# arihantb2/direct_lidar_odometry

Hardware: AMD Instinct MI355X
Metric: gicp_iterations_per_sec (higher is better)
Workload: dtype f64

## Files before the change

### direct_lidar_odometry_amd/csrc/ngicp_align.h

```cpp
#pragma once

namespace {

std::mutex& persist_mutex(int device) {
  static std::mutex m[64];
  return m[(unsigned)device % 64u];
}

int pass_impl() {
  static const int impl = std::getenv("NGICP_PASS_IMPL") ? std::atoi(std::getenv("NGICP_PASS_IMPL")) : 0;
  return impl;
}

const char* robust_unsupported_switch(const ngicp* h) {
  if (pass_impl() == 1) return "NGICP_PASS_IMPL=1";
  if (const char* s = std::getenv("NGICP_FUSED")) if (std::atoi(s) != 0) return "NGICP_FUSED";
  if (const char* s = std::getenv("NGICP_QUEUE")) if (std::atoi(s) != 0) return "NGICP_QUEUE";
  if (h->persist) return "NGICP_PERSIST";
  if (h->head) return "NGICP_HEAD";
  return nullptr;
}
void refuse_if_robust(const ngicp* h, const char* entry) {
  if (h->robust_kind != NGICP_ROBUST_NONE)
    throw ArgError{NGICP_ERR_ARG, std::string(entry) + ": not available with a robust kernel set (ngicp_set_robust_kernel(h, NGICP_ROBUST_NONE, 0) turns it off)"};
// ... 164 lines not shown
  s.partials = a.partials;
  s.nblocks = nblocks;
  s.grp_order = order_buf[h->order_sel];
  s.grp_cost = a.grp_cost;
  s.trace = own_buffers ? h->trace.as<double>() : nullptr;
  s.max_trace_rows = max_rows;
  s.mode = 0;
  s.sums_out = nullptr;
  s.dbg_stamps = nullptr;
  s.progress_host = nullptr;
  s.final_host = nullptr;
  s.order_valid = order_flag[h->order_sel];
  s.t_first = nullptr;
  s.persist = 0;
  s.pass_honours_word = 0;
  s.pass_ticks = nullptr;
  s.st_out = nullptr;
  s.nrows = 0;
  a.crow_in = nullptr;
  a.crow_out = nullptr;
  a.cluster_ticket = nullptr;
  a.done_flag = nullptr;
  c.nblocks = nblocks;
  if (!own_buffers) return;
  h->stats.lanes_per_query = 2;
  h->stats.voxel_size = a.grid.h;
  h->stats.grid_dims[0] = a.grid.nx;
  h->stats.grid_dims[1] = a.grid.ny;
  h->stats.grid_dims[2] = a.grid.nz;
}
// ... 387 lines not shown
    HIP_TRY(hipMemsetAsync(c.pa.ticket, 0, sizeof(int), h->stream));
  }
  const long max_p = max_passes(h->p);
  const bool plain = h->p.max_iter > 0 && pass_impl() == 0 && !c.pa.fused && !xcd_order && !dbg.span_path && !dbg.qstat_path && !c.sa.dbg_stamps;
  const bool want_persist = h->persist && plain && h->persist_slots > 0 && !dbg.stamp_path && max_p + 1 <= kMaxPersistPasses;
  const bool persist_done = want_persist && align_persistent(h, c, al, max_p);
  const bool head_mode = h->head && plain && !persist_done && c.nblocks <= 2 * h->pass_slots;
  if (persist_done) {
  } else if (head_mode) {
    head_begin(h);
    feed_alignment(h, al, max_p + 1, [&](long i, hipEvent_t start, hipEvent_t stop) { launch_head(h, c, i, start, stop); });
    if ((al.st.hot.passes + 1) & 1) HIP_TRY(hipMemcpyAsync(h->state.p, h->state_alt.p, sizeof(LmState), hipMemcpyDeviceToDevice, h->stream));
  } else if (persist_one && h->persist_slots > 0 && max_p + 1 <= kMaxPersistPasses) {
    feed_alignment(h, al, max_p, [&](long i, hipEvent_t start, hipEvent_t stop) { launch_persist_one(h, c, i, start, stop); });
  } else {
    feed_alignment(h, al, max_p, [&](long, hipEvent_t start, hipEvent_t stop) {
      launch_pass(h, c.pa, c.nblocks, h->stream, start, stop);
      if (!c.pa.fused) hipLaunchKernelGGL(k_lm_solve, dim3(1), dim3(kSolveThreads), 0, h->stream, c.sa);
    });
  }
  HIP_TRY(hipGetLastError());
  debug_end(h, c, dbg);
  end_alignment(h, al, aligned, out_stride, !persist_done);
  ngicp_stats& s = h->stats;
  h->order_src = h->src.dev.get();
  h->order_groups = c.sa.nblocks;
  s.staged_fraction = al.st.hot.search_passes > 0 ? al.st.hot.staged_total / ((double)al.st.hot.search_passes * (double)h->src.dev->n) : 0.0;
  if (al.st.hot.search_passes > 1) h->prev_staged_fraction = s.staged_fraction;
  if (persist_done && h->profiling) sum_tick_pass_times(h, al.st.hot);
}

struct VoxelCtx {
  VoxelPassArgs pa;
// ... 354 lines not shown
```

### direct_lidar_odometry_amd/csrc/ngicp_api.hip

```cpp
#include "../../include/ngicp.h"

#include <hip/hip_runtime.h>
#include <hip/hip_ext.h>

#include <algorithm>
#include <atomic>
#include <chrono>
#include <cmath>
#include <cstdio>
#include <cstdlib>
#include <cstring>
#include <limits>
#include <memory>
#include <mutex>
#include <sched.h>
#include <string>
#include <vector>

#include "ngicp_pass.h"
#include "ngicp_cloudops.h"
#include "ngicp_filters.h"
#include "ngicp_query.h"
#include "ngicp_range.h"
#include "ngicp_batch.h"
// ... 544 lines not shown
      HIP_TRY(hipDeviceGetAttribute(&cus, hipDeviceAttributeMultiprocessorCount, device));
      HIP_TRY(hipOccupancyMaxActiveBlocksPerMultiprocessor(&per_cu, k_gicp_pass<2, 3>, 256, 0));
      h->pass_slots = std::max(1, cus) * std::max(1, per_cu);
      int per_cu_p = 0;
      if (hipOccupancyMaxActiveBlocksPerMultiprocessor(&per_cu_p, k_gicp_persist<2, 3>, 256, 0) == hipSuccess) h->persist_slots = std::max(0, cus) * std::max(0, per_cu_p);
      int q3 = 0, q4 = 0;
      if (hipOccupancyMaxActiveBlocksPerMultiprocessor(&q3, k_gicp_queue<2, 3>, 256, 0) == hipSuccess && q3 > 0) h->queue_slots[0] = cus * q3;
      if (hipOccupancyMaxActiveBlocksPerMultiprocessor(&q4, k_gicp_queue<2, 4>, 256, 0) == hipSuccess && q4 > 0) h->queue_slots[1] = cus * q4;
      int coop = 0;
      if (hipDeviceGetAttribute(&coop, hipDeviceAttributeCooperativeLaunch, device) != hipSuccess || !coop) h->persist_slots = 0;
    }
    HIP_TRY(hipHostMalloc(reinterpret_cast<void**>(&h->pin_ticks), 2 * kMaxTickPasses * sizeof(unsigned long long), hipHostMallocDefault));
    if (const char* s = std::getenv("NGICP_PERSIST")) h->persist = std::atoi(s);
    if (const char* s = std::getenv("NGICP_HEAD")) h->head = std::atoi(s);
    if (const char* s = std::getenv("NGICP_FULL_LAST_PASS")) h->full_last_pass = std::atoi(s);
    if (const char* s = std::getenv("NGICP_CELL_BOXES")) h->cell_boxes = std::atoi(s);
    if (const char* s = std::getenv("NGICP_TARGET_OCC")) h->target_occupancy = std::max(1.0, std::atof(s));
    if (const char* s = std::getenv("NGICP_VOXEL")) h->voxel_size = std::atof(s);
    if (const char* s = std::getenv("NGICP_CHUNK")) h->chunk_pairs = std::max(1, std::min(64, std::atoi(s)));
    if (const char* s = std::getenv("NGICP_STAGE_GROW")) h->stage_grow = std::max(0, std::min(kStageMaxGrow, std::atoi(s)));
    {
      HandleRegistry& r = registry();
      std::lock_guard<std::mutex> lock(r.m);
      r.live.push_back(h.get());
    }
    *out = h.release();
    return NGICP_OK;
  } catch (const HipError& e) {
    g_create_error = std::string("HIP error in ") + e.what + ": " + hipGetErrorString(e.code);
    (void)hipGetLastError();
// ... 1141 lines not shown
  return guarded(h, [&] {
    static const int kIn[4] = {3, 42, 6, 6}, kOut[4] = {9, 6, 12, 6};
    if (which < 0 || which > 3 || !in || !out) throw ArgError{NGICP_ERR_ARG, "bad arguments"};
    if (n_problems == 0) return;
    DevBuf di, dout;
    di.ensure(n_problems * kIn[which] * sizeof(double));
    dout.ensure(n_problems * kOut[which] * sizeof(double));
    HIP_TRY(hipMemcpyAsync(di.p, in, n_problems * kIn[which] * sizeof(double), hipMemcpyHostToDevice, h->stream));
    hipLaunchKernelGGL(k_math_selftest, dim3((unsigned)((n_problems + 63) / 64)), dim3(64), 0, h->stream, which, di.as<double>(), (int)n_problems, dout.as<double>());
    HIP_TRY(hipMemcpyAsync(out, dout.p, n_problems * kOut[which] * sizeof(double), hipMemcpyDeviceToHost, h->stream));
    HIP_TRY(hipStreamSynchronize(h->stream));
    HIP_TRY(hipGetLastError());
  });
}

int ngicp_measure_copy_bandwidth(ngicp_t* h, size_t bytes, int reps, double* gbps_out) {
  return guarded(h, [&] {
    if (!gbps_out || bytes < 4096 || reps <= 0) throw ArgError{NGICP_ERR_ARG, "bad arguments"};
    const size_t n16 = bytes / 16;
    DevBuf a, b;
    a.ensure(n16 * 16);
    b.ensure(n16 * 16);
    HIP_TRY(hipMemsetAsync(a.p, 1, n16 * 16, h->stream));
    const unsigned blocks = (unsigned)((n16 + 1023) / 1024);
    for (int i = 0; i < 2; ++i) hipLaunchKernelGGL(k_stream_copy, dim3(blocks), dim3(256), 0, h->stream, a.as<float4>(), b.as<float4>(), n16);
    HIP_TRY(hipEventRecord(h->ev_a, h->stream));
    for (int i = 0; i < reps; ++i) hipLaunchKernelGGL(k_stream_copy, dim3(blocks), dim3(256), 0, h->stream, a.as<float4>(), b.as<float4>(), n16);
    HIP_TRY(hipEventRecord(h->ev_b, h->stream));
    HIP_TRY(hipEventSynchronize(h->ev_b));
    float ms = 0.f;
// ... 140 lines not shown
```

### direct_lidar_odometry_amd/csrc/ngicp_handle.h

```cpp
#pragma once

namespace {

thread_local std::string g_create_error;

struct HipError {
  hipError_t code;
  const char* what;
  const char* file;
  int line;
};

#define HIP_TRY(expr)                                          \
  do {                                                         \
    hipError_t _e = (expr);                                    \
    if (_e != hipSuccess) throw HipError{_e, #expr, __FILE__, __LINE__}; \
  } while (0)

struct ArgError {
  int code;
  std::string msg;
};

double now_ms() {
// ... 242 lines not shown

  Slot src, tgt;
  CovSet src_covs, tgt_covs;

  DevBuf raw, unsorted, keys, counts, fill, tile_sums, tile_sq, tmp, bbox, occ;
  int pass_slots = 768;
  int persist_slots = 0;
  int queue_slots[2] = {768, 1024};
  int persist = 0;
  int order_sel = 0;
  DevBuf grp_order_alt;
  DevBuf gen_lines;
  int cell_boxes = 0;
  int head = 0;
  int full_last_pass = 0;
  DevBuf state_alt;
  DevBuf head_ws;
  unsigned long long* pin_ticks = nullptr;
  double prev_staged_fraction = -1.0;
  DevBuf dbg, dbg_q, dbg_s, dbg_span, grp_order, grp_cost, batch_far;
  const void* order_src = nullptr;
  int order_groups = -1;
  DevBuf tpt[2], mahal[2], partials, state, trace, tfinal, out_xyz, scratch16, queries, knn_idx, knn_d2, sums, ticket;
  DevBuf fit_T, fit_part, fit_out, rad_counts, rad_offsets, rad_keys, rad_long;
  size_t rad_total = 0;
  bool rad_valid = false;
  DevBuf range_ws;
  hipEvent_t ev_q_a = nullptr, ev_q_b = nullptr;
  std::vector<hipEvent_t> prof_events;
  int* h_progress = nullptr;
// ... 124 lines not shown
```

### direct_lidar_odometry_amd/csrc/ngicp_math.h

```cpp
#pragma once
#include <hip/hip_runtime.h>
#include <math.h>

#define NG_HD __host__ __device__ __forceinline__

namespace ngk {

struct Pose {
  double R[9];
  double t[3];
};

NG_HD void pose_identity(Pose& p) {
  for (int i = 0; i < 9; ++i) p.R[i] = (i % 4 == 0) ? 1.0 : 0.0;
  p.t[0] = p.t[1] = p.t[2] = 0.0;
}

NG_HD void pose_mul(const Pose& a, const Pose& b, Pose& c) {
#pragma unroll
  for (int i = 0; i < 3; ++i) {
#pragma unroll
    for (int j = 0; j < 3; ++j) c.R[i * 3 + j] = a.R[i * 3 + 0] * b.R[0 * 3 + j] + a.R[i * 3 + 1] * b.R[1 * 3 + j] + a.R[i * 3 + 2] * b.R[2 * 3 + j];
    c.t[i] = a.R[i * 3 + 0] * b.t[0] + a.R[i * 3 + 1] * b.t[1] + a.R[i * 3 + 2] * b.t[2] + a.t[i];
  }
}

NG_HD void so3_exp_matrix(const double w[3], double R[9]) {
  const double theta_sq = w[0] * w[0] + w[1] * w[1] + w[2] * w[2];
  double imag, real;
  if (theta_sq < 1e-10) {
    const double theta_quad = theta_sq * theta_sq;
    imag = 0.5 - 1.0 / 48.0 * theta_sq + 1.0 / 3840.0 * theta_quad;
    real = 1.0 - 1.0 / 8.0 * theta_sq + 1.0 / 384.0 * theta_quad;
  } else {
    const double theta = sqrt(theta_sq);
    const double half = 0.5 * theta;
    imag = sin(half) / theta;
    real = cos(half);
// ... 97 lines not shown
        p = i;
      }
    }
    piv[k] = p;
#pragma unroll
    for (int i = k + 1; i < 6; ++i)
      if (p == i) {
#pragma unroll
        for (int j = 0; j < 6; ++j) NG_SWAP(A[k * 6 + j], A[i * 6 + j]);
#pragma unroll
        for (int j = 0; j < 6; ++j) NG_SWAP(A[j * 6 + k], A[j * 6 + i]);
      }
    const double dk = A[k * 6 + k];
    if (dk != 0.0 && isfinite(dk)) {
#pragma unroll
      for (int i = k + 1; i < 6; ++i) A[i * 6 + k] /= dk;
#pragma unroll
      for (int i = k + 1; i < 6; ++i)
#pragma unroll
        for (int j = k + 1; j <= i; ++j) {
          A[i * 6 + j] -= A[i * 6 + k] * dk * A[j * 6 + k];
          A[j * 6 + i] = A[i * 6 + j];
        }
    }
  }
  double y[6];
#pragma unroll
  for (int i = 0; i < 6; ++i) y[i] = rhs[i];
#pragma unroll
  for (int k = 0; k < 6; ++k)
#pragma unroll
    for (int i = k + 1; i < 6; ++i)
      if (piv[k] == i) NG_SWAP(y[k], y[i]);
#pragma unroll
  for (int i = 0; i < 6; ++i)
#pragma unroll
    for (int j = 0; j < i; ++j) y[i] -= A[i * 6 + j] * y[j];
  const double tol = 2.2250738585072014e-308;
#pragma unroll
  for (int i = 0; i < 6; ++i) y[i] = (fabs(A[i * 6 + i]) > tol) ? y[i] / A[i * 6 + i] : 0.0;
#pragma unroll
  for (int i = 5; i >= 0; --i)
#pragma unroll
    for (int j = i + 1; j < 6; ++j) y[i] -= A[j * 6 + i] * y[j];
#pragma unroll
  for (int k = 5; k >= 0; --k)
#pragma unroll
    for (int i = k + 1; i < 6; ++i)
      if (piv[k] == i) NG_SWAP(y[k], y[i]);
#pragma unroll
  for (int i = 0; i < 6; ++i) x[i] = y[i];
}
#undef NG_SWAP

}
```

### direct_lidar_odometry_amd/csrc/ngicp_pass.h

```cpp
#pragma once
#include <type_traits>

#include "../../include/ngicp.h"
#include "ngicp_knn.h"

namespace ngk {

constexpr int kPartialStride = 32;
constexpr int kNumSums = 29;
constexpr int kNumSlots = 32;
constexpr int kTraceCols = 8;

__device__ __forceinline__ void lin_terms(double (&acc)[kNumSums], const double tax, const double tay, const double taz, const double ex, const double ey, const double ez,
                                          const double (&M)[6]) {
  const double m00 = M[0], m01 = M[1], m02 = M[2], m11 = M[3], m12 = M[4], m22 = M[5];
  const double mex = m00 * ex + m01 * ey + m02 * ez;
  const double mey = m01 * ex + m11 * ey + m12 * ez;
  const double mez = m02 * ex + m12 * ey + m22 * ez;
  acc[27] += ex * mex + ey * mey + ez * mez;
  const double A00 = tay * m02 - taz * m01, A10 = taz * m00 - tax * m02, A20 = tax * m01 - tay * m00;
  const double A01 = tay * m12 - taz * m11, A11 = taz * m01 - tax * m12, A21 = tax * m11 - tay * m01;
  const double A02 = tay * m22 - taz * m12, A12 = taz * m02 - tax * m22, A22 = tax * m12 - tay * m02;
  acc[0] += -(A01 * taz - A02 * tay);
  acc[1] += -(-A00 * taz + A02 * tax);
// ... 169 lines not shown
  double* trace;
  int max_trace_rows;
  int mode;
  double* sums_out;
  int* grp_order;
  const int* grp_cost;
  unsigned long long* dbg_stamps;
  int* progress_host;
  LmHot* final_host;
  int* order_valid;
  const unsigned long long* t_first;
  LmState* st_out;
  int nrows;
  int persist;
  int pass_honours_word;
  unsigned long long* pass_ticks;
};

struct PassArgs {
  const float4* qpts;
  const int2* batches;
  const float* batch_boxes;
  const int* grp_order;
  int* grp_cost;
  int n_batches;
  const double* cov_src;
  int n_src;
  const float4* tgt;
  const float4* tgtp;
  const Xyz* tgt3;
  const int* tgt_cell_start;
  const unsigned int* tgt_cell_box;
// ... 297 lines not shown

constexpr int kSolveRowSubsets = 32;
constexpr int kProgressDone = 1 << 30, kProgressMask = kProgressDone - 1;

__device__ __forceinline__ bool is_converged_dev(const Pose& d, double rot_eps, double trans_eps) {
  double rmax = 0.0, tmax = 0.0;
#pragma unroll
  for (int r = 0; r < 3; ++r) {
#pragma unroll
    for (int c = 0; c < 3; ++c) rmax = fmax(rmax, 1.0 / rot_eps * fabs(d.R[r * 3 + c] - (r == c ? 1.0 : 0.0)));
    tmax = fmax(tmax, 1.0 / trans_eps * fabs(d.t[r]));
  }
  return fmax(rmax, tmax) < 1;
}

__device__ __forceinline__ void make_trial(LmHot& L, double lambda_add) {
  double A[36], rhs[6];
#pragma unroll
  for (int i = 0; i < 36; ++i) A[i] = L.H[i];
#pragma unroll
  for (int i = 0; i < 6; ++i) {
    A[i * 6 + i] += lambda_add;
    rhs[i] = -L.b[i];
  }
  ldlt6_solve(A, rhs, L.d);
  pose_identity(L.delta);
  so3_exp_matrix(L.d, L.delta.R);
  L.delta.t[0] = L.d[3];
  L.delta.t[1] = L.d[4];
  L.delta.t[2] = L.d[5];
// ... 49 lines not shown
      for (int i = 0; i < 6; ++i) m = fmax(m, fabs(L.H[i * 6 + i]));
      L.lambda = cfg.lm_init_lambda_factor * m;
    }
    L.nu = 2.0;
    L.trial = 0;
    if (cfg.lm_max_iterations <= 0) {
      L.lm_failed = 1;
      L.done = 1;
      return false;
    }
    make_trial(L, L.lambda);
    set_lin_unneeded(L, cfg);
    return false;
  }

  double den = 0.0, dn = 0.0;
#pragma unroll
  for (int i = 0; i < 6; ++i) {
    den += L.d[i] * (L.lambda * L.d[i] - L.b[i]);
    dn += L.d[i] * L.d[i];
  }
  const double rho = (L.y0 - yi) / den;
  const bool rejected = rho < 0;
  if (trace && L.n_trace < max_trace_rows) {
    double* row = trace + (size_t)L.n_trace * kTraceCols;
    row[0] = L.iter; row[1] = L.trial; row[2] = L.y0; row[3] = yi;
    row[4] = rho; row[5] = L.lambda; row[6] = sqrt(dn); row[7] = rejected ? 0.0 : 1.0;
    L.n_trace += 1;
  }
  if (rejected) {
    if (is_converged_dev(L.delta, cfg.rot_eps, cfg.trans_eps)) {
      L.converged = 1;
      L.done = 1;
      return false;
    }
    L.lambda = L.nu * L.lambda;
// ... 8 lines not shown
    make_trial(L, L.lambda);
    set_lin_unneeded(L, cfg);
    return false;
  }
  return true;
}

__device__ __forceinline__ void lm_step(LmHot& L, const LmConfig& cfg, const double* sums, double* trace, int max_trace_rows, const bool searched = true) {
  const bool gn = cfg.optimizer == 0;
  L.search_passes += searched ? 1 : 0;
  const bool accepted = lm_advance(L, cfg, sums, trace, max_trace_rows);
  if (accepted) {
#pragma unroll
    for (int i = 0; i < 36; ++i) L.final_H[i] = L.H[i];
    if (!gn) {
      double den = 0.0;
#pragma unroll
      for (int i = 0; i < 6; ++i) den += L.d[i] * (L.lambda * L.d[i] - L.b[i]);
      const double rho = (L.y0 - sums[28]) / den;
      L.x0 = L.xi;
      const double q = 2 * rho - 1;
      L.lambda = L.lambda * fmax(1.0 / 3.0, 1 - q * q * q);
      L.converged = is_converged_dev(L.delta, cfg.rot_eps, cfg.trans_eps) ? 1 : 0;
      L.iter += 1;
      if (L.converged || L.iter >= cfg.max_iterations) {
        L.done = 1;
      } else {
        adopt_new(L, sums);
        L.nr_iterations = L.iter;
        L.nu = 2.0;
        L.trial = 0;
        make_trial(L, L.lambda);
        set_lin_unneeded(L, cfg);
      }
    }
  }
  if (gn && !L.done) L.xi = L.x0;
}

template <int THREADS>
struct SolveShared {
  double wsum[32][kPartialStride];
  double sums[kPartialStride];
  int ord_cnt[THREADS / 64 - 1][16], ord_pos[THREADS / 64 - 1][16];
  int ord_cost[kMaxOrderGroups];
  unsigned char ord_cls[kMaxOrderGroups];
  int ord_arrived;
  LmHot L;
};

template <int THREADS, bool AGENT, bool PERSIST = false>
__device__ __forceinline__ void lm_solve_body(const SolveArgs& a, SolveShared<THREADS>& sh) {
// ... 188 lines not shown
        const int base = ord_pos[sw][cls];
        if (valid) a.grp_order[base + __popcll(m & lt)] = gi;
        wsync();
        if (valid && (m & lt) == 0) ord_pos[sw][cls] = base + __popcll(m);
        wsync();
      }
      if (sw == 0 && lane == 0 && a.order_valid) *a.order_valid = 1;
    }
    if (a.dbg_stamps && sw == 0 && lane == 0) a.dbg_stamps[7] = __builtin_amdgcn_s_memtime() - t_ord;
  }
  if (wave != 0) return;
  if (a.mode == 2) {
    if (lane == 0) st->hot.y0 = sums[28];
    return;
  }
  if (lane == 0) {
    if (a.mode == 1) {
      adopt_new(L, sums);
    } else {
      const LmConfig& cfg = a.cfg;
      NG_SSTAMP(3);
      lm_step(L, cfg, sums, a.trace, a.max_trace_rows, !(a.pass_honours_word && L.lin_unneeded));
      NG_SSTAMP(4);
      NG_SSTAMP(5);
      if (!L.done) {
#pragma unroll
        for (int r = 0; r < 3; ++r) {
#pragma unroll
          for (int c = 0; c < 4; ++c) {
            const float f = (float)(c < 3 ? L.xi.R[r * 3 + c] : L.xi.t[r]);
            if constexpr (PERSIST) __hip_atomic_store(&st->xi_f[r * 4 + c], f, __ATOMIC_RELAXED, __HIP_MEMORY_SCOPE_AGENT);
// ... 36 lines not shown
    } else if (lane == kViewCur) {
      v = L.cur;
    } else if (lane == kViewHaveLin) {
      v = L.have_lin;
    }
    __hip_atomic_store(st->view + (size_t)L.passes * kViewWords + lane, v, __ATOMIC_RELAXED, __HIP_MEMORY_SCOPE_AGENT);
  }
  NG_SSTAMP(6);
#undef NG_SSTAMP
}

__global__ void __launch_bounds__(kSolveThreads) k_lm_solve(SolveArgs a) {
  __shared__ SolveShared<kSolveThreads> sh;
  lm_solve_body<kSolveThreads, false>(a, sh);
}

constexpr int kStampStride = 24;
#define NG_STAMP(k)                                                                                   \
  do {                                                                                                \
    if (a.dbg_stamps && lane == 0) a.dbg_stamps[(size_t)(blockIdx.x * 4 + wave) * kStampStride + (k)] = __builtin_amdgcn_s_memtime(); \
  } while (0)

template <int G, int WPS = NGICP_PASS_WAVES, bool FUSED = false, bool ROBUST = false>
__global__ void __launch_bounds__(256, WPS) k_gicp_pass(PassArgs a) {
  constexpr int B = 64 / G;
  constexpr int kWin = WPS >= 4 ? 12 : 16, kSideStep = WPS >= 4 ? 8 : 16;
  static_assert(kWin <= kSortedPad, "walk windows may overhang the array by at most the sentinel frame");
  static_assert(B == kBatchQueries, "query batches are built for 32 queries (2 lanes per query)");
  __shared__ double lds[4][kNumSlots];
  struct Nothing {};
// ... 460 lines not shown
```

### direct_lidar_odometry_amd/nano_gicp.py

```python
from __future__ import annotations

import ctypes as C
import enum
import os
import sys

import numpy as np

_HERE = os.path.dirname(os.path.abspath(__file__))
_LIB_PATH = os.environ.get("NGICP_LIB") or os.path.join(_HERE, "libngicp_hip.so")

c_f32p = C.POINTER(C.c_float)
c_f64p = C.POINTER(C.c_double)
c_i32p = C.POINTER(C.c_int)

FLT_MAX = float(np.finfo(np.float32).max)


class RegularizationMethod(enum.IntEnum):
    NONE = 0
    MIN_EIG = 1
    NORMALIZED_MIN_EIG = 2
    PLANE = 3
    FROBENIUS = 4
# ... 37 lines not shown
        return d


EXPORTS = [
    "ngicp_create", "ngicp_destroy", "ngicp_last_error", "ngicp_version", "ngicp_set_params", "ngicp_set_tuning",
    "ngicp_set_source", "ngicp_register_source", "ngicp_set_target", "ngicp_clear_source", "ngicp_clear_target",
    "ngicp_share_source_index", "ngicp_swap_source_target", "ngicp_compute_source_covs", "ngicp_compute_target_covs",
    "ngicp_copy_source_covs", "ngicp_clear_source_covs", "ngicp_clear_target_covs", "ngicp_source_covs_size",
    "ngicp_target_covs_size", "ngicp_get_source_covs", "ngicp_get_target_covs", "ngicp_set_source_covs",
    "ngicp_set_target_covs", "ngicp_align", "ngicp_linearize", "ngicp_compute_error", "ngicp_get_correspondences",
    "ngicp_target_knn", "ngicp_get_lm_trace", "ngicp_get_stats", "ngicp_set_profiling", "ngicp_sharded_begin",
    "ngicp_sharded_pass", "ngicp_sharded_step", "ngicp_sharded_finish",
    "ngicp_keyframe_add", "ngicp_keyframe_add_transformed", "ngicp_keyframe_add_transformed_filtered", "ngicp_keyframe_count", "ngicp_keyframe_size", "ngicp_keyframe_clear",
    "ngicp_submap_set", "ngicp_get_target_points", "ngicp_transform_source", "ngicp_transform_cloud", "ngicp_measure_copy_bandwidth",
    "ngicp_preprocess_scan", "ngicp_set_source_preprocessed", "ngicp_map_add", "ngicp_map_voxel_filter", "ngicp_map_size", "ngicp_map_get",
    "ngicp_map_clear", "ngicp_math_selftest", "ngicp_set_host_wait", "ngicp_covs_shard_begin", "ngicp_covs_shard_compute", "ngicp_covs_shard_commit",
    "ngicp_knn_search", "ngicp_radius_search", "ngicp_radius_fetch", "ngicp_fitness_score",
    "ngicp_align_batch", "ngicp_batch_get_lm_trace", "ngicp_fitness_score_batch",
    "ngicp_range_select", "ngicp_range_median",
    "ngicp_set_voxel_resolution", "ngicp_voxelmap_size", "ngicp_voxelmap_get",
    "ngicp_set_voxel_neighbors", "ngicp_get_voxel_neighbors", "ngicp_voxel_correspondences", "ngicp_voxelmap_builds",
    "ngicp_voxel_align_batch",
    "ngicp_set_voxel_submap_merge", "ngicp_get_voxel_submap_merge", "ngicp_voxelmap_merge_stats", "ngicp_keyframe_voxelmap_get",
    "ngicp_set_voxel_rolling", "ngicp_get_voxel_rolling", "ngicp_voxel_rolling_insert", "ngicp_voxel_rolling_evict", "ngicp_voxel_rolling_clear",
    "ngicp_voxel_rolling_get", "ngicp_voxel_rolling_stats",
    "ngicp_set_robust_kernel", "ngicp_get_robust_kernel", "ngicp_robust_terms",
]

BATCH_MAX_LANES = 64

_lib = None
# ... 62 lines not shown
    L.ngicp_keyframe_size.argtypes = [vp, C.c_int, C.POINTER(C.c_size_t)]
    L.ngicp_keyframe_clear.argtypes = [vp]
    L.ngicp_submap_set.argtypes = [vp, c_i32p, C.c_size_t, c_i32p]
    L.ngicp_get_target_points.argtypes = [vp, c_f32p, C.c_size_t, C.POINTER(C.c_size_t)]
    L.ngicp_transform_source.argtypes = [vp, c_f32p, c_f32p, C.c_size_t]
    L.ngicp_transform_cloud.argtypes = [vp, c_f32p, C.c_size_t, C.c_size_t, c_f32p, c_f32p, C.c_size_t]
    L.ngicp_measure_copy_bandwidth.argtypes = [vp, C.c_size_t, C.c_int, c_f64p]
    L.ngicp_preprocess_scan.argtypes = [vp, c_f32p, C.c_size_t, C.c_size_t, C.c_long, C.c_int, C.c_float, C.c_float, c_f32p, C.c_size_t, C.POINTER(C.c_size_t)]
    L.ngicp_set_source_preprocessed.argtypes = [vp, C.c_uint64]
    L.ngicp_map_add.argtypes = [vp, c_f32p, C.c_size_t, C.c_size_t, C.c_long]
    L.ngicp_map_voxel_filter.argtypes = [vp, C.c_float, C.POINTER(C.c_size_t)]
    L.ngicp_map_size.argtypes = [vp, C.POINTER(C.c_size_t)]
    L.ngicp_map_get.argtypes = [vp, c_f32p, C.c_size_t]
    L.ngicp_map_clear.argtypes = [vp]
    L.ngicp_math_selftest.argtypes = [vp, C.c_int, c_f64p, C.c_size_t, c_f64p]
    L.ngicp_set_voxel_resolution.argtypes = [vp, C.c_double]
    L.ngicp_voxelmap_size.argtypes = [vp, C.POINTER(C.c_size_t)]
    L.ngicp_voxelmap_get.argtypes = [vp, c_i32p, c_f64p, c_f64p, c_i32p]
    L.ngicp_set_voxel_neighbors.argtypes = [vp, C.c_int]
    L.ngicp_get_voxel_neighbors.argtypes = [vp, c_i32p]
    L.ngicp_voxel_correspondences.argtypes = [vp, c_i32p, C.c_size_t, c_i32p]
    L.ngicp_voxelmap_builds.argtypes = [vp, C.POINTER(C.c_longlong)]
    L.ngicp_set_voxel_submap_merge.argtypes = [vp, C.c_int]
    L.ngicp_get_voxel_submap_merge.argtypes = [vp, c_i32p]
    L.ngicp_voxelmap_merge_stats.argtypes = [vp, C.POINTER(C.c_longlong), C.POINTER(C.c_longlong), c_f64p, c_f64p]
    L.ngicp_keyframe_voxelmap_get.argtypes = [vp, C.c_int, C.POINTER(C.c_size_t), c_i32p, c_f64p, c_f64p, c_i32p]
    c_i64p, c_szp = C.POINTER(C.c_longlong), C.POINTER(C.c_size_t)
    L.ngicp_set_voxel_rolling.argtypes = [vp, C.c_int]
    L.ngicp_get_voxel_rolling.argtypes = [vp, c_i32p]
    L.ngicp_voxel_rolling_insert.argtypes = [vp, vp, c_f32p, c_szp, c_szp]
# ... 511 lines not shown
    def mapGet(self) -> np.ndarray:
        n = self.mapSize()
        out = np.empty((n, 4), dtype=np.float32)
        if n:
            self._ck(self._L.ngicp_map_get(self._h, _p(out, c_f32p), n))
        return out

    def mapClear(self): self._ck(self._L.ngicp_map_clear(self._h))

    def mathSelftest(self, which: int, problems) -> np.ndarray:
        a = np.ascontiguousarray(problems, dtype=np.float64)
        out = np.empty((a.shape[0], (9, 6, 12, 6)[which]))
        self._ck(self._L.ngicp_math_selftest(self._h, int(which), _p(a, c_f64p), a.shape[0], _p(out, c_f64p)))
        return out

    def measureCopyBandwidth(self, nbytes: int = 1 << 30, reps: int = 10) -> float:
        v = C.c_double(0)
        self._ck(self._L.ngicp_measure_copy_bandwidth(self._h, int(nbytes), int(reps), C.byref(v)))
        return v.value

    def covsShardBegin(self, which: int):
        ptr = C.c_void_p(0); n = C.c_size_t(0)
        self._ck(self._L.ngicp_covs_shard_begin(self._h, int(which), C.byref(ptr), C.byref(n)))
        return ptr.value, n.value

    def covsShardCompute(self, which: int, lo: int, hi: int, stream: int = 0):
        self._ck(self._L.ngicp_covs_shard_compute(self._h, int(which), int(lo), int(hi), C.c_void_p(stream) if stream else None))

    def covsShardCommit(self, which: int):
        self._ck(self._L.ngicp_covs_shard_commit(self._h, int(which)))
# ... 34 lines not shown
```

### include/ngicp.h

```cpp
#ifndef NGICP_H
#define NGICP_H

#include <stddef.h>
#include <stdint.h>

#ifdef __cplusplus
extern "C" {
#endif

typedef struct ngicp ngicp_t;

#define NGICP_OK 0
#define NGICP_ERR_HIP (-1)
#define NGICP_ERR_ARG (-2)
#define NGICP_ERR_STATE (-3)
#define NGICP_ERR_K_TOO_LARGE (-4)

#define NGICP_REG_NONE 0
#define NGICP_REG_MIN_EIG 1
#define NGICP_REG_NORMALIZED_MIN_EIG 2
#define NGICP_REG_PLANE 3
#define NGICP_REG_FROBENIUS 4

#define NGICP_OPT_GAUSS_NEWTON 0
// ... 71 lines not shown
#define NGICP_ROBUST_CAUCHY 2
#define NGICP_ROBUST_GEMAN_MCCLURE 3
int ngicp_set_robust_kernel(ngicp_t* h, int kind, double width);
int ngicp_get_robust_kernel(const ngicp_t* h, int* kind, double* width);
int ngicp_robust_terms(ngicp_t* h, const double T_colmajor[16], double* s_out, double* w_out, size_t capacity_doubles, int* K_out);

#define NGICP_BATCH_MAX_LANES 64
int ngicp_align_batch(ngicp_t* h, size_t n_guesses, const float* guesses_n16_colmajor, float* T_out_n16_colmajor, int* converged_n, int* nr_iterations_n,
                      double* final_hessians_n36_colmajor_or_null);
int ngicp_voxel_align_batch(ngicp_t* h, size_t n_guesses, const float* guesses_n16_colmajor, float* T_out_n16_colmajor, int* converged_n, int* nr_iterations_n,
                            double* final_hessians_n36_colmajor_or_null);
int ngicp_batch_get_lm_trace(ngicp_t* h, size_t lane, double* rows8_or_null, size_t max_rows, size_t* n_rows);
int ngicp_fitness_score_batch(ngicp_t* h, size_t n, const float* T_n16_colmajor, double max_range, double* scores_n, size_t* n_inliers_n_or_null);

int ngicp_math_selftest(ngicp_t* h, int which, const double* in, size_t n_problems, double* out);

typedef struct ngicp_stats {
  double align_ms;
  double loop_ms;
  double pass_ms_total;
  int passes;
  int outer_iterations;
  int lm_trials;
  double mean_candidates;
  double valid_fraction;
  double index_build_ms;
  double covariance_ms;
  double upload_ms;
  double voxel_size;
  int grid_dims[3];
// ... 51 lines not shown
```

Baseline: 20480.

## Run the LM step and 6x6 solve across a wavefront instead of lane 0

```diff
diff --git a/direct_lidar_odometry_amd/csrc/ngicp_align.h b/direct_lidar_odometry_amd/csrc/ngicp_align.h
--- a/direct_lidar_odometry_amd/csrc/ngicp_align.h
+++ b/direct_lidar_odometry_amd/csrc/ngicp_align.h
@@ -202,6 +202,7 @@
   s.t_first = nullptr;
   s.persist = 0;
   s.pass_honours_word = 0;
+  s.serial_step = h->serial_step;
   s.pass_ticks = nullptr;
   s.st_out = nullptr;
   s.nrows = 0;
@@ -619,9 +620,13 @@
   } else if (persist_one && h->persist_slots > 0 && max_p + 1 <= kMaxPersistPasses) {
     feed_alignment(h, al, max_p, [&](long i, hipEvent_t start, hipEvent_t stop) { launch_persist_one(h, c, i, start, stop); });
   } else {
-    feed_alignment(h, al, max_p, [&](long, hipEvent_t start, hipEvent_t stop) {
+    static const long stamp_launch = std::getenv("NGICP_DEBUG_SOLVE") ? std::atol(std::getenv("NGICP_DEBUG_SOLVE")) : 0;
+    feed_alignment(h, al, max_p, [&](long i, hipEvent_t start, hipEvent_t stop) {
       launch_pass(h, c.pa, c.nblocks, h->stream, start, stop);
-      if (!c.pa.fused) hipLaunchKernelGGL(k_lm_solve, dim3(1), dim3(kSolveThreads), 0, h->stream, c.sa);
+      if (c.pa.fused) return;
+      SolveArgs sa = c.sa;
+      if (stamp_launch > 1 && i + 1 != stamp_launch) sa.dbg_stamps = nullptr;
+      hipLaunchKernelGGL(k_lm_solve, dim3(1), dim3(kSolveThreads), 0, h->stream, sa);
     });
   }
   HIP_TRY(hipGetLastError());
diff --git a/direct_lidar_odometry_amd/csrc/ngicp_api.hip b/direct_lidar_odometry_amd/csrc/ngicp_api.hip
--- a/direct_lidar_odometry_amd/csrc/ngicp_api.hip
+++ b/direct_lidar_odometry_amd/csrc/ngicp_api.hip
@@ -582,6 +582,7 @@
     if (const char* s = std::getenv("NGICP_PERSIST")) h->persist = std::atoi(s);
     if (const char* s = std::getenv("NGICP_HEAD")) h->head = std::atoi(s);
     if (const char* s = std::getenv("NGICP_FULL_LAST_PASS")) h->full_last_pass = std::atoi(s);
+    if (const char* s = std::getenv("NGICP_SERIAL_STEP")) h->serial_step = std::atoi(s) != 0 ? 1 : 0;
     if (const char* s = std::getenv("NGICP_CELL_BOXES")) h->cell_boxes = std::atoi(s);
     if (const char* s = std::getenv("NGICP_TARGET_OCC")) h->target_occupancy = std::max(1.0, std::atof(s));
     if (const char* s = std::getenv("NGICP_VOXEL")) h->voxel_size = std::atof(s);
@@ -1753,6 +1754,25 @@
   });
 }
 
+int ngicp_step_selftest(ngicp_t* h, const double* in, size_t n_problems, unsigned char* out_or_null, size_t* record_bytes) {
+  return guarded(h, [&] {
+    if (record_bytes) *record_bytes = kStepSelftestRecord;
+    if (!out_or_null) return;
+    if (!in || n_problems > (size_t)1 << 20) throw ArgError{NGICP_ERR_ARG, "bad arguments"};
+    if (n_problems == 0) return;
+    DevBuf di, dout;
+    const size_t in_bytes = n_problems * kStepSelftestIn * sizeof(double), out_bytes = n_problems * 2 * kStepSelftestRecord;
+    di.ensure(in_bytes);
+    dout.ensure(out_bytes);
+    HIP_TRY(hipMemcpyAsync(di.p, in, in_bytes, hipMemcpyHostToDevice, h->stream));
+    HIP_TRY(hipMemsetAsync(dout.p, 0, out_bytes, h->stream));
+    hipLaunchKernelGGL(k_step_selftest, dim3((unsigned)n_problems), dim3(64), 0, h->stream, di.as<double>(), (int)n_problems, dout.as<unsigned char>());
+    HIP_TRY(hipMemcpyAsync(out_or_null, dout.p, out_bytes, hipMemcpyDeviceToHost, h->stream));
+    HIP_TRY(hipStreamSynchronize(h->stream));
+    HIP_TRY(hipGetLastError());
+  });
+}
+
 int ngicp_measure_copy_bandwidth(ngicp_t* h, size_t bytes, int reps, double* gbps_out) {
   return guarded(h, [&] {
     if (!gbps_out || bytes < 4096 || reps <= 0) throw ArgError{NGICP_ERR_ARG, "bad arguments"};
diff --git a/direct_lidar_odometry_amd/csrc/ngicp_handle.h b/direct_lidar_odometry_amd/csrc/ngicp_handle.h
--- a/direct_lidar_odometry_amd/csrc/ngicp_handle.h
+++ b/direct_lidar_odometry_amd/csrc/ngicp_handle.h
@@ -280,6 +280,7 @@
   int cell_boxes = 0;
   int head = 0;
   int full_last_pass = 0;
+  int serial_step = 0;
   DevBuf state_alt;
   DevBuf head_ws;
   unsigned long long* pin_ticks = nullptr;
diff --git a/direct_lidar_odometry_amd/csrc/ngicp_math.h b/direct_lidar_odometry_amd/csrc/ngicp_math.h
--- a/direct_lidar_odometry_amd/csrc/ngicp_math.h
+++ b/direct_lidar_odometry_amd/csrc/ngicp_math.h
@@ -16,12 +16,19 @@
   p.t[0] = p.t[1] = p.t[2] = 0.0;
 }
 
+NG_HD double pose_mul_r(double a0, double a1, double a2, double b0, double b1, double b2) { return a0 * b0 + a1 * b1 + a2 * b2; }
+NG_HD double pose_mul_t(double a0, double a1, double a2, double b0, double b1, double b2, double t) { return a0 * b0 + a1 * b1 + a2 * b2 + t; }
+NG_HD double ldlt_scale(double a_ik, double dk) { return a_ik / dk; }
+NG_HD double ldlt_update(double a_ij, double a_ik, double dk, double a_jk) { return a_ij - a_ik * dk * a_jk; }
+NG_HD double ldlt_subst(double y_i, double a, double y_j) { return y_i - a * y_j; }
+NG_HD double ldlt_diag(double y_i, double a_ii) { return (fabs(a_ii) > 2.2250738585072014e-308) ? y_i / a_ii : 0.0; }
+
 NG_HD void pose_mul(const Pose& a, const Pose& b, Pose& c) {
 #pragma unroll
   for (int i = 0; i < 3; ++i) {
 #pragma unroll
-    for (int j = 0; j < 3; ++j) c.R[i * 3 + j] = a.R[i * 3 + 0] * b.R[0 * 3 + j] + a.R[i * 3 + 1] * b.R[1 * 3 + j] + a.R[i * 3 + 2] * b.R[2 * 3 + j];
-    c.t[i] = a.R[i * 3 + 0] * b.t[0] + a.R[i * 3 + 1] * b.t[1] + a.R[i * 3 + 2] * b.t[2] + a.t[i];
+    for (int j = 0; j < 3; ++j) c.R[i * 3 + j] = pose_mul_r(a.R[i * 3 + 0], a.R[i * 3 + 1], a.R[i * 3 + 2], b.R[0 * 3 + j], b.R[1 * 3 + j], b.R[2 * 3 + j]);
+    c.t[i] = pose_mul_t(a.R[i * 3 + 0], a.R[i * 3 + 1], a.R[i * 3 + 2], b.t[0], b.t[1], b.t[2], a.t[i]);
   }
 }
 
@@ -149,12 +156,12 @@
     const double dk = A[k * 6 + k];
     if (dk != 0.0 && isfinite(dk)) {
 #pragma unroll
-      for (int i = k + 1; i < 6; ++i) A[i * 6 + k] /= dk;
+      for (int i = k + 1; i < 6; ++i) A[i * 6 + k] = ldlt_scale(A[i * 6 + k], dk);
 #pragma unroll
       for (int i = k + 1; i < 6; ++i)
 #pragma unroll
         for (int j = k + 1; j <= i; ++j) {
-          A[i * 6 + j] -= A[i * 6 + k] * dk * A[j * 6 + k];
+          A[i * 6 + j] = ldlt_update(A[i * 6 + j], A[i * 6 + k], dk, A[j * 6 + k]);
           A[j * 6 + i] = A[i * 6 + j];
         }
     }
@@ -170,14 +177,13 @@
 #pragma unroll
   for (int i = 0; i < 6; ++i)
 #pragma unroll
-    for (int j = 0; j < i; ++j) y[i] -= A[i * 6 + j] * y[j];
-  const double tol = 2.2250738585072014e-308;
+    for (int j = 0; j < i; ++j) y[i] = ldlt_subst(y[i], A[i * 6 + j], y[j]);
 #pragma unroll
-  for (int i = 0; i < 6; ++i) y[i] = (fabs(A[i * 6 + i]) > tol) ? y[i] / A[i * 6 + i] : 0.0;
+  for (int i = 0; i < 6; ++i) y[i] = ldlt_diag(y[i], A[i * 6 + i]);
 #pragma unroll
   for (int i = 5; i >= 0; --i)
 #pragma unroll
-    for (int j = i + 1; j < 6; ++j) y[i] -= A[j * 6 + i] * y[j];
+    for (int j = i + 1; j < 6; ++j) y[i] = ldlt_subst(y[i], A[j * 6 + i], y[j]);
 #pragma unroll
   for (int k = 5; k >= 0; --k)
 #pragma unroll
diff --git a/direct_lidar_odometry_amd/csrc/ngicp_pass.h b/direct_lidar_odometry_amd/csrc/ngicp_pass.h
--- a/direct_lidar_odometry_amd/csrc/ngicp_pass.h
+++ b/direct_lidar_odometry_amd/csrc/ngicp_pass.h
@@ -207,8 +207,11 @@
   int nrows;
   int persist;
   int pass_honours_word;
+  int serial_step;
   unsigned long long* pass_ticks;
 };
+
+static_assert(offsetof(SolveArgs, pass_ticks) == offsetof(SolveArgs, pass_honours_word) + 8, "serial_step takes no room of its own");
 
 struct PassArgs {
   const float4* qpts;
@@ -536,6 +539,23 @@
   return fmax(rmax, tmax) < 1;
 }
 
+__device__ __forceinline__ double lm_gain_den(const double* d, const double* b, const double lambda) {
+  double den = 0.0;
+#pragma unroll
+  for (int i = 0; i < 6; ++i) den += d[i] * (lambda * d[i] - b[i]);
+  return den;
+}
+__device__ __forceinline__ double lm_step_norm2(const double* d) {
+  double dn = 0.0;
+#pragma unroll
+  for (int i = 0; i < 6; ++i) dn += d[i] * d[i];
+  return dn;
+}
+__device__ __forceinline__ double lm_lambda_accepted(const double lambda, const double rho) {
+  const double q = 2 * rho - 1;
+  return lambda * fmax(1.0 / 3.0, 1 - q * q * q);
+}
+
 __device__ __forceinline__ void make_trial(LmHot& L, double lambda_add) {
   double A[36], rhs[6];
 #pragma unroll
@@ -615,12 +635,7 @@
     return false;
   }
 
-  double den = 0.0, dn = 0.0;
-#pragma unroll
-  for (int i = 0; i < 6; ++i) {
-    den += L.d[i] * (L.lambda * L.d[i] - L.b[i]);
-    dn += L.d[i] * L.d[i];
-  }
+  const double den = lm_gain_den(L.d, L.b, L.lambda), dn = lm_step_norm2(L.d);
   const double rho = (L.y0 - yi) / den;
   const bool rejected = rho < 0;
   if (trace && L.n_trace < max_trace_rows) {
@@ -659,13 +674,9 @@
 #pragma unroll
     for (int i = 0; i < 36; ++i) L.final_H[i] = L.H[i];
     if (!gn) {
-      double den = 0.0;
-#pragma unroll
-      for (int i = 0; i < 6; ++i) den += L.d[i] * (L.lambda * L.d[i] - L.b[i]);
-      const double rho = (L.y0 - sums[28]) / den;
+      const double rho = (L.y0 - sums[28]) / lm_gain_den(L.d, L.b, L.lambda);
       L.x0 = L.xi;
-      const double q = 2 * rho - 1;
-      L.lambda = L.lambda * fmax(1.0 / 3.0, 1 - q * q * q);
+      L.lambda = lm_lambda_accepted(L.lambda, rho);
       L.converged = is_converged_dev(L.delta, cfg.rot_eps, cfg.trans_eps) ? 1 : 0;
       L.iter += 1;
       if (L.converged || L.iter >= cfg.max_iterations) {
@@ -681,6 +692,237 @@
     }
   }
   if (gn && !L.done) L.xi = L.x0;
+}
+
+__device__ __forceinline__ void wave_sync() {
+  __builtin_amdgcn_fence(__ATOMIC_RELEASE, "wavefront");
+  __builtin_amdgcn_wave_barrier();
+  __builtin_amdgcn_fence(__ATOMIC_ACQUIRE, "wavefront");
+}
+__device__ __forceinline__ double wave_lane_f64(const double v, const int src_lane) {
+  return __hiloint2double(__builtin_amdgcn_readlane(__double2hiint(v), src_lane), __builtin_amdgcn_readlane(__double2loint(v), src_lane));
+}
+__device__ __forceinline__ double wave_fetch_f64(const double v, const int src_lane) {
+  return __hiloint2double(__builtin_amdgcn_ds_bpermute(src_lane << 2, __double2hiint(v)), __builtin_amdgcn_ds_bpermute(src_lane << 2, __double2loint(v)));
+}
+__device__ __forceinline__ bool wave_agree(const bool b) { return __builtin_amdgcn_readfirstlane(b ? 1 : 0) != 0; }
+__device__ __forceinline__ int pose_elem_to_rows(const int e) { return e < 9 ? (e / 3) * 4 + e % 3 : (e - 9) * 4 + 3; }
+
+__device__ __forceinline__ void adopt_new_wave(LmHot& L, const double* sums, const int lane) {
+  if (lane < 36) {
+    const int i = lane / 6, j = lane - 6 * i;
+    L.H[lane] = sums[tri21(min(i, j), max(i, j))];
+  }
+  if (lane < 6) L.b[lane] = sums[21 + lane];
+  if (lane < 12) L.lin_f[pose_elem_to_rows(lane)] = (float)reinterpret_cast<const double*>(&L.xi)[lane];
+  if (lane == 0) {
+    L.y0 = sums[27];
+    L.cur ^= 1;
+    L.have_lin = 1;
+  }
+}
+
+__device__ __forceinline__ void make_trial_wave(LmHot& L, const LmConfig& cfg, const double lambda_add, const bool lin_word, const int iter, const int lane) {
+  wave_sync();
+  const bool act = lane < 36;
+  const int i = act ? lane / 6 : 0, j = act ? lane - 6 * i : 0;
+  const int r = max(i, j), c = min(i, j);
+  double a = act ? L.H[lane] : 0.0;
+  if (act && i == j) a += lambda_add;
+  double y[6];
+#pragma unroll
+  for (int e = 0; e < 6; ++e) y[e] = -L.b[e];
+  const bool out_t = lane >= 9;
+  const int orow = lane < 12 ? (out_t ? lane - 9 : lane / 3) : 0, ocol = lane < 9 ? lane % 3 : 0;
+  double xb[3];
+#pragma unroll
+  for (int m = 0; m < 3; ++m) xb[m] = out_t ? L.x0.t[m] : L.x0.R[m * 3 + ocol];
+  int piv[6];
+#pragma unroll
+  for (int k = 0; k < 6; ++k) {
+    int p = k;
+    double best = fabs(wave_lane_f64(a, 7 * k));
+#pragma unroll
+    for (int q = k + 1; q < 6; ++q) {
+      const double v = fabs(wave_lane_f64(a, 7 * q));
+      if (v > best) {
+        best = v;
+        p = q;
+      }
+    }
+    p = __builtin_amdgcn_readfirstlane(p);
+    piv[k] = p;
+    if (p != k) {
+      const int si = i == k ? p : (i == p ? k : i), sj = j == k ? p : (j == p ? k : j);
+      a = wave_fetch_f64(a, si * 6 + sj);
+    }
+    if (k < 5) {
+      const double dk = wave_lane_f64(a, 7 * k);
+      if (dk != 0.0 && isfinite(dk)) {
+        const double scaled = ldlt_scale(a, dk);
+        if (act && j == k && i > k) a = scaled;
+        const double upd = ldlt_update(wave_fetch_f64(a, r * 6 + c), wave_fetch_f64(a, r * 6 + k), dk, wave_fetch_f64(a, c * 6 + k));
+        if (act && i > k && j > k) a = upd;
+      }
+    }
+  }
+#pragma unroll
+  for (int k = 0; k < 6; ++k)
+#pragma unroll
+    for (int q = k + 1; q < 6; ++q)
+      if (piv[k] == q) {
+        const double t = y[k];
+        y[k] = y[q];
+        y[q] = t;
+      }
+  double lo[15];
+#pragma unroll
+  for (int q = 1; q < 6; ++q)
+#pragma unroll
+    for (int e = 0; e < q; ++e) lo[q * (q - 1) / 2 + e] = wave_lane_f64(a, q * 6 + e);
+#pragma unroll
+  for (int q = 0; q < 6; ++q)
+#pragma unroll
+    for (int e = 0; e < q; ++e) y[q] = ldlt_subst(y[q], lo[q * (q - 1) / 2 + e], y[e]);
+  {
+    double mine = y[0];
+#pragma unroll
+    for (int q = 1; q < 6; ++q) mine = lane == 7 * q ? y[q] : mine;
+    const double dv = ldlt_diag(mine, a);
+#pragma unroll
+    for (int q = 0; q < 6; ++q) y[q] = wave_lane_f64(dv, 7 * q);
+  }
+#pragma unroll
+  for (int q = 5; q >= 0; --q)
+#pragma unroll
+    for (int e = q + 1; e < 6; ++e) y[q] = ldlt_subst(y[q], lo[e * (e - 1) / 2 + q], y[e]);
+#pragma unroll
+  for (int k = 5; k >= 0; --k)
+#pragma unroll
+    for (int q = k + 1; q < 6; ++q)
+      if (piv[k] == q) {
+        const double t = y[k];
+        y[k] = y[q];
+        y[q] = t;
+      }
+  Pose delta;
+  so3_exp_matrix(y, delta.R);
+  delta.t[0] = y[3];
+  delta.t[1] = y[4];
+  delta.t[2] = y[5];
+  double ar[3];
+#pragma unroll
+  for (int m = 0; m < 3; ++m) ar[m] = orow == 0 ? delta.R[m] : (orow == 1 ? delta.R[3 + m] : delta.R[6 + m]);
+  const double at = orow == 0 ? delta.t[0] : (orow == 1 ? delta.t[1] : delta.t[2]);
+  const double xr = pose_mul_r(ar[0], ar[1], ar[2], xb[0], xb[1], xb[2]), xt = pose_mul_t(ar[0], ar[1], ar[2], xb[0], xb[1], xb[2], at);
+  if (lane < 12) reinterpret_cast<double*>(&L.xi)[lane] = out_t ? xt : xr;
+  const bool conv = lin_word ? is_converged_dev(delta, cfg.rot_eps, cfg.trans_eps) : false;
+  if (lane == 0) {
+#pragma unroll
+    for (int e = 0; e < 6; ++e) L.d[e] = y[e];
+    L.delta = delta;
+    if (lin_word) L.lin_unneeded = (conv || iter + 1 >= cfg.max_iterations) ? 1 : 0;
+  }
+}
+
+__device__ __forceinline__ void lm_step_wave(LmHot& L, const LmConfig& cfg, const double* sums, double* trace, int max_trace_rows, const bool searched, const int lane) {
+  const double yi = sums[28];
+  int iter = L.iter;
+  double lambda = L.lambda;
+  const int have_lin = L.have_lin;
+  if (lane == 0) {
+    L.search_passes += searched ? 1 : 0;
+    L.passes += 1;
+    L.cand_total += sums[29];
+    L.valid_total += sums[30];
+    L.staged_total += sums[31];
+  }
+  const bool gn = cfg.optimizer == 0;
+  bool go_on = true;
+  if (gn) {
+    adopt_new_wave(L, sums, lane);
+    lambda = 0.0;
+  } else if (!wave_agree(have_lin != 0)) {
+    adopt_new_wave(L, sums, lane);
+    if (wave_agree(lambda < 0.0)) {
+      double m = 0.0;
+#pragma unroll
+      for (int i = 0; i < 6; ++i) m = fmax(m, fabs(sums[tri21(i, i)]));
+      lambda = cfg.lm_init_lambda_factor * m;
+    }
+    go_on = cfg.lm_max_iterations > 0;
+    if (lane == 0) {
+      L.nr_iterations = 0;
+      L.lambda = lambda;
+      L.nu = 2.0;
+      L.trial = 0;
+      if (!go_on) L.lm_failed = 1, L.done = 1;
+    }
+  } else {
+    double d[6], b[6];
+#pragma unroll
+    for (int e = 0; e < 6; ++e) d[e] = L.d[e], b[e] = L.b[e];
+    const double y0 = L.y0, nu = L.nu;
+    const int trial = L.trial, n_trace = L.n_trace;
+    const double rho = (y0 - yi) / lm_gain_den(d, b, lambda);
+    const bool rejected = wave_agree(rho < 0);
+    if (trace && n_trace < max_trace_rows && lane == 0) {
+      double* row = trace + (size_t)n_trace * kTraceCols;
+      row[0] = iter; row[1] = trial; row[2] = y0; row[3] = yi;
+      row[4] = rho; row[5] = lambda; row[6] = sqrt(lm_step_norm2(d)); row[7] = rejected ? 0.0 : 1.0;
+      L.n_trace = n_trace + 1;
+    }
+    const bool conv = wave_agree(is_converged_dev(L.delta, cfg.rot_eps, cfg.trans_eps));
+    if (rejected) {
+      const bool failed = !conv && trial + 1 >= cfg.lm_max_iterations;
+      go_on = !conv && !failed;
+      if (!conv) lambda = nu * lambda;
+      if (lane == 0) {
+        if (conv) {
+          L.converged = 1, L.done = 1;
+        } else {
+          L.lambda = lambda;
+          L.nu = 2 * nu;
+          L.trial = trial + 1;
+          if (failed) L.lm_failed = 1, L.converged = 0, L.done = 1;
+        }
+      }
+    } else {
+      if (lane < 36) L.final_H[lane] = L.H[lane];
+      if (lane < 12) reinterpret_cast<double*>(&L.x0)[lane] = reinterpret_cast<const double*>(&L.xi)[lane];
+      lambda = lm_lambda_accepted(lambda, rho);
+      iter += 1;
+      go_on = !(conv || iter >= cfg.max_iterations);
+      if (lane == 0) {
+        L.lambda = lambda;
+        L.converged = conv ? 1 : 0;
+        L.iter = iter;
+        if (!go_on) L.done = 1;
+      }
+      if (go_on) {
+        adopt_new_wave(L, sums, lane);
+        if (lane == 0) {
+          L.nr_iterations = iter;
+          L.nu = 2.0;
+          L.trial = 0;
+        }
+      }
+    }
+  }
+  if (!wave_agree(go_on)) return;
+  make_trial_wave(L, cfg, lambda, !gn, iter, lane);
+  if (gn) {
+    wave_sync();
+    if (lane < 12) reinterpret_cast<double*>(&L.x0)[lane] = reinterpret_cast<const double*>(&L.xi)[lane];
+    if (lane < 36) L.final_H[lane] = L.H[lane];
+    const bool conv = wave_agree(is_converged_dev(L.delta, cfg.rot_eps, cfg.trans_eps));
+    if (lane == 0) {
+      L.nr_iterations = iter;
+      L.converged = conv ? 1 : 0;
+      L.iter = iter + 1;
+      if (conv || iter + 1 >= cfg.max_iterations) L.done = 1;
+    }
+  }
 }
 
 template <int THREADS>
@@ -899,7 +1141,18 @@
     if (lane == 0) st->hot.y0 = sums[28];
     return;
   }
-  if (lane == 0) {
+  if (a.mode != 1 && !a.serial_step) {
+    NG_SSTAMP(3);
+    lm_step_wave(L, a.cfg, sums, a.trace, a.max_trace_rows, !(a.pass_honours_word && L.lin_unneeded), lane);
+    NG_SSTAMP(4);
+    wave_sync();
+    NG_SSTAMP(5);
+    if (!L.done && lane < 12) {
+      const float f = (float)reinterpret_cast<const double*>(&L.xi)[lane];
+      if constexpr (PERSIST) __hip_atomic_store(&st->xi_f[pose_elem_to_rows(lane)], f, __ATOMIC_RELAXED, __HIP_MEMORY_SCOPE_AGENT);
+      else sto->xi_f[pose_elem_to_rows(lane)] = f;
+    }
+  } else if (lane == 0) {
     if (a.mode == 1) {
       adopt_new(L, sums);
     } else {
@@ -966,6 +1219,59 @@
   __shared__ SolveShared<kSolveThreads> sh;
   lm_solve_body<kSolveThreads, false>(a, sh);
 }
+
+constexpr int kStepSelftestIn = 132;
+constexpr size_t kStepSelftestRecord = sizeof(LmHot) + 18 * sizeof(double);
+static_assert(sizeof(LmHot) % 8 == 0, "the trace row behind the image is 8-byte aligned");
+__global__ void __launch_bounds__(64) k_step_selftest(const double* __restrict__ in, int n_problems, unsigned char* __restrict__ out) {
+  __shared__ LmHot L;
+  __shared__ double sums[kPartialStride];
+  static_assert(kPartialStride >= 32, "32 reduced sums");
+  const int lane = threadIdx.x;
+  if ((int)blockIdx.x >= n_problems) return;
+  const double* p = in + (size_t)blockIdx.x * kStepSelftestIn;
+  LmConfig cfg;
+  cfg.max_iterations = (int)p[93];
+  cfg.lm_max_iterations = (int)p[94];
+  cfg.optimizer = (int)p[95];
+  cfg.rot_eps = p[96];
+  cfg.trans_eps = p[97];
+  cfg.lm_init_lambda_factor = p[98];
+  const bool searched = p[131] != 0.0;
+  for (int form = 0; form < 2; ++form) {
+    unsigned char* rec = out + ((size_t)blockIdx.x * 2 + form) * kStepSelftestRecord;
+    double* tail = reinterpret_cast<double*>(rec + sizeof(LmHot));
+    __syncthreads();
+    for (int w = lane; w < (int)(sizeof(LmHot) / 4); w += 64) reinterpret_cast<int*>(&L)[w] = 0;
+    if (lane < 32) sums[lane] = p[99 + lane];
+    __syncthreads();
+    if (lane < 36) reinterpret_cast<double*>(&L.x0)[lane] = p[lane];
+    if (lane < 36) L.H[lane] = p[36 + lane];
+    if (lane < 6) L.b[lane] = p[72 + lane], L.d[lane] = p[79 + lane];
+    if (lane == 0) {
+      L.y0 = p[78];
+      L.lambda = p[85];
+      L.nu = p[86];
+      L.iter = (int)p[87];
+      L.trial = (int)p[88];
+      L.have_lin = (int)p[89];
+      L.cur = (int)p[90];
+      L.n_trace = max(0, (int)p[91]);
+      L.lin_unneeded = (int)p[92];
+    }
+    __syncthreads();
+    if (form == 0) {
+      if (lane == 0) lm_step(L, cfg, sums, tail, 1, searched);
+    } else {
+      lm_step_wave(L, cfg, sums, tail, 1, searched, lane);
+    }
+    __syncthreads();
+    for (int w = lane; w < (int)(sizeof(LmHot) / 4); w += 64) reinterpret_cast<int*>(rec)[w] = reinterpret_cast<const int*>(&L)[w];
+    if (lane < 6) tail[8 + lane] = L.d[lane];
+    if (lane == 0) tail[14] = L.done, tail[15] = L.converged, tail[16] = L.lm_failed, tail[17] = L.trial;
+  }
+}
+static_assert(offsetof(LmHot, xi) == offsetof(LmHot, x0) + sizeof(Pose) && offsetof(LmHot, delta) == offsetof(LmHot, xi) + sizeof(Pose), "x0, xi, delta are contiguous");
 
 constexpr int kStampStride = 24;
 #define NG_STAMP(k)                                                                                   \
diff --git a/direct_lidar_odometry_amd/nano_gicp.py b/direct_lidar_odometry_amd/nano_gicp.py
--- a/direct_lidar_odometry_amd/nano_gicp.py
+++ b/direct_lidar_odometry_amd/nano_gicp.py
@@ -75,7 +75,7 @@
     "ngicp_keyframe_add", "ngicp_keyframe_add_transformed", "ngicp_keyframe_add_transformed_filtered", "ngicp_keyframe_count", "ngicp_keyframe_size", "ngicp_keyframe_clear",
     "ngicp_submap_set", "ngicp_get_target_points", "ngicp_transform_source", "ngicp_transform_cloud", "ngicp_measure_copy_bandwidth",
     "ngicp_preprocess_scan", "ngicp_set_source_preprocessed", "ngicp_map_add", "ngicp_map_voxel_filter", "ngicp_map_size", "ngicp_map_get",
-    "ngicp_map_clear", "ngicp_math_selftest", "ngicp_set_host_wait", "ngicp_covs_shard_begin", "ngicp_covs_shard_compute", "ngicp_covs_shard_commit",
+    "ngicp_map_clear", "ngicp_math_selftest", "ngicp_step_selftest", "ngicp_set_host_wait", "ngicp_covs_shard_begin", "ngicp_covs_shard_compute", "ngicp_covs_shard_commit",
     "ngicp_knn_search", "ngicp_radius_search", "ngicp_radius_fetch", "ngicp_fitness_score",
     "ngicp_align_batch", "ngicp_batch_get_lm_trace", "ngicp_fitness_score_batch",
     "ngicp_range_select", "ngicp_range_median",
@@ -168,6 +168,7 @@
     L.ngicp_map_get.argtypes = [vp, c_f32p, C.c_size_t]
     L.ngicp_map_clear.argtypes = [vp]
     L.ngicp_math_selftest.argtypes = [vp, C.c_int, c_f64p, C.c_size_t, c_f64p]
+    L.ngicp_step_selftest.argtypes = [vp, c_f64p, C.c_size_t, C.POINTER(C.c_ubyte), C.POINTER(C.c_size_t)]
     L.ngicp_set_voxel_resolution.argtypes = [vp, C.c_double]
     L.ngicp_voxelmap_size.argtypes = [vp, C.POINTER(C.c_size_t)]
     L.ngicp_voxelmap_get.argtypes = [vp, c_i32p, c_f64p, c_f64p, c_i32p]
@@ -709,6 +710,16 @@
         self._ck(self._L.ngicp_math_selftest(self._h, int(which), _p(a, c_f64p), a.shape[0], _p(out, c_f64p)))
         return out
 
+    def stepSelftest(self, problems) -> np.ndarray:
+        a = np.ascontiguousarray(problems, dtype=np.float64)
+        assert a.ndim == 2 and a.shape[1] == 132
+        rec = C.c_size_t(0)
+        self._ck(self._L.ngicp_step_selftest(self._h, None, 0, None, C.byref(rec)))
+        out = np.zeros((a.shape[0], 2, rec.value), dtype=np.uint8)
+        if a.shape[0]:
+            self._ck(self._L.ngicp_step_selftest(self._h, _p(a, c_f64p), a.shape[0], _p(out, C.POINTER(C.c_ubyte)), C.byref(rec)))
+        return out
+
     def measureCopyBandwidth(self, nbytes: int = 1 << 30, reps: int = 10) -> float:
         v = C.c_double(0)
         self._ck(self._L.ngicp_measure_copy_bandwidth(self._h, int(nbytes), int(reps), C.byref(v)))
diff --git a/include/ngicp.h b/include/ngicp.h
--- a/include/ngicp.h
+++ b/include/ngicp.h
@@ -109,6 +109,7 @@
 int ngicp_fitness_score_batch(ngicp_t* h, size_t n, const float* T_n16_colmajor, double max_range, double* scores_n, size_t* n_inliers_n_or_null);
 
 int ngicp_math_selftest(ngicp_t* h, int which, const double* in, size_t n_problems, double* out);
+int ngicp_step_selftest(ngicp_t* h, const double* in, size_t n_problems, unsigned char* out_or_null, size_t* record_bytes);
 
 typedef struct ngicp_stats {
   double align_ms;
```

After: 20970 (median of 6 runs). +2.4%, better.
